# TongtongSong/OpenEAT

Measured on AMD Instinct MI355X. Metric: audio-frames/sec/GPU (train) + RTF (attention-rescoring decode), 12L Conformer, higher is better.
Workload: dtype f32 (storage, accumulate, softmax, norms, losses, optimizer all fp32; every matrix product is the fp32 product to within one fp32 rounding, computed as six exact bf16 x bf16 MFMA products of three-piece operand splits h+m+l = x, dropped terms < 2^-24 |a||b| - tests hold it to the exact-fp32 mode's t; 1 GPU; configs[1]: 12L Conformer d=256 (12+3+3, h=4, ff=1024, K=15, V=3246), B=32/GPU x 10 s 16 kHz wav (T=998 frames), L=30, CTC+attention joint loss, fbank+fwd+bwd+clip+Adam, dropout 0.1; global_batch=32, parallelism=dp1, hip_graph=True

## Files before the change

### include/openeat_hip.h

```cpp
#ifndef OPENEAT_HIP_H
#define OPENEAT_HIP_H

#include <stddef.h>
#include <stdint.h>

#ifdef __cplusplus
extern "C" {
#endif

const char* oe_last_error(void);
int oe_abi_version(void);

int oe_capture_unjoined_streams(void* origin, void* const* sides, int n_sides, int* unjoined_index);

int oe_stamp(long long* buf, int slot, void* stream);

enum { OE_GATHER_NONE = 0, OE_GATHER_A = 1, OE_GATHER_B = 2 };

typedef struct oe_gemm_args {
    const float* a; long lda; int a_kmajor;
    const float* b; long ldb; int b_kmajor;
    float* c; long ldc;
    int m, n, k;
    int split_k;
// ... 160 lines not shown
    const float* d_out;
    float* dq; float* dk; float* dv;
    float* dkeybias;
    float* delta;
    int precision;
    int causal;
} oe_attn_args;

int oe_attention_fwd(const oe_attn_args* args, void* stream);
int oe_attention_bwd(const oe_attn_args* args, void* stream);

int oe_relpos_prepare(const float* k, long k_bstride, long k_rstride, const float* p, long p_rstride,
                      const float* u, const float* v, int B, int T, int H, int D, float scale, float* kp,
                      float* keybias, void* stream);
int oe_relpos_backward(const float* dkp, const float* dkeybias, const float* k, long k_bstride, long k_rstride,
                       const float* p, long p_rstride, const float* u, const float* v, int B, int T, int H, int D,
                       float scale, float* dk, float* dp, long dp_rstride, float* du, float* dv, void* stream);

int oe_glu_fwd(const float* a, long rows, int d, float* y, void* stream);
int oe_glu_bwd(const float* a, const float* dy, long rows, int d, float* da, void* stream);

int oe_dropout_scale(const float* x, long n, int cols, float alpha, float p, unsigned long long seed,
                     const unsigned long long* seed_dev, const unsigned char* rowmask, float* out, void* stream);

int oe_embed_fwd(const long long* tokens, const float* table, const float* pe, long rows, int L, int d, int V,
                 float xscale, float* out, void* stream);
int oe_embed_bwd(const long long* tokens, const float* dout, long rows, int d, int V, float xscale, float* dtable,
                 void* stream);

int oe_swap_last2(const float* in, long A, int Bd, int Cd, float* out, int accumulate, void* stream);
int oe_pad1_nhwc(const float* dy, int B, int To, int Fo, int C, float* out, void* stream);
int oe_pad1_nhwc_planes(const float* dy, int B, int To, int Fo, int C, float* out, void* planes, long plane_stride, void* stream);
int oe_conv_dgrad_k3s2_weights(const float* w, int C, float* out, void* stream);

int oe_loss_combine(const float* loss_ctc, const float* loss_att, const float* loss_att_r, float ctc_weight, float reverse_weight,
                    float inv_accum, float* out, void* stream);
int oe_loss_combine_bwd(const float* g, float ctc_weight, float reverse_weight, float inv_accum, float* d_ctc, float* d_att,
                        float* d_att_r, void* stream);

int oe_axpby(const float* x, const float* y, long n, float a, float b, const float* a_dev, float* out, void* stream);

int oe_act_fwd(const float* x, long n, int act, float* y, void* stream);
int oe_act_grad(const float* dy, const float* pre, long n, int act, float* out, void* stream);

int oe_log_softmax(const float* x, long rows, int V, float* out, void* stream);
int oe_logprob_gather(const float* x, long rows, int V, const long long* idx_a, int idx_b, float* out_a, float* out_b, void* stream);
int oe_att_inputs(const int* ys_pad, const int* ys_lens, int B, int L, int sos, int eos, int ignore_id, long long* ys_in,
                  long long* ys_out, long long* r_ys_in, long long* r_ys_out, unsigned char* tgt_mask, void* stream);
int oe_topk_rows(const float* x, long rows, int V, int k, int log_softmax, float* vals, long long* idx, void* stream);

int oe_masked_softmax_fwd(const float* scores, const unsigned char* mask, long mask_bstride, long mask_rstride, int B, int H,
                          int T1, int T2, float drop_p, unsigned long long seed, const unsigned long long* seed_dev, float* y,
                          float* out, void* stream);
int oe_masked_softmax_bwd(const float* y, const float* dout, long rows, int T2, float drop_p, unsigned long long seed,
                          const unsigned long long* seed_dev, float* dscores, void* stream);

int oe_global_cmvn(const float* x, const float* mean, const float* istd, long n, int F, float* y, void* stream);

int oe_conv1_fwd(const float* x, const float* w, const float* bias, int B, int T, int F, int C, float* y, void* stream);
int oe_conv1_fwd_pl(const float* x, const float* w, const float* bias, int B, int T, int F, int C, float* y,
                    void* y_planes, long plane_stride, void* stream);
int oe_conv1_wgrad(const float* x, const float* dy, int B, int T, int F, int C, float* dw, float* db, void* stream);

int oe_col2im_relu(const float* dcol, const float* y1, int B, int T1, int F1, int C, float* dx, void* stream);
int oe_col2im_relu_ks(const float* dcol, const float* y1, int B, int T1, int F1, int C, int KS, int S, float* dx,
                      void* stream);
// ... 100 lines not shown
```

### openeat_amd/csrc/conv.hip

```cpp
#include <stdlib.h>
#include "oe_common.h"
#include "../../include/openeat_hip.h"

__global__ __launch_bounds__(256) void conv1_fwd_kernel(const float* __restrict__ x, const float* __restrict__ w,
                                                         const float* __restrict__ bias, int B, int T, int F, int T1, int F1,
                                                         int C, int pos_per_block, float* __restrict__ y,
                                                         __bf16* __restrict__ y_planes, long plane_stride) {
    const int cpt = C >> 2;
    const int grp = threadIdx.x / cpt;
    const int c4 = (threadIdx.x % cpt) * 4;
    const int ngrp = blockDim.x / cpt;
    float wr[4][9], br[4];
#pragma unroll
    for (int e = 0; e < 4; ++e) {
        br[e] = bias[c4 + e];
#pragma unroll
        for (int k = 0; k < 9; ++k) wr[e][k] = w[(c4 + e) * 9 + k];
    }
    const long npos = (long)B * T1 * F1;
    const long p0 = (long)blockIdx.x * pos_per_block;
    for (long pos = p0 + grp; pos < min(npos, p0 + pos_per_block); pos += ngrp) {
        const int f = (int)(pos % F1);
        const int t = (int)((pos / F1) % T1);
        const long b = pos / ((long)F1 * T1);
// ... 524 lines not shown
    hipLaunchKernelGGL(pad1_nhwc_planes_kernel, dim3((unsigned)min((long)oe_cdiv(n, 256), 65536L)), dim3(256), 0, (hipStream_t)stream,
                       (const float4*)dy, B, To, Fo, C / 4, (float4*)out, (__bf16*)planes, plane_stride);
    OE_LAUNCH_CHECK("pad1_nhwc_planes");
    return 0;
}
__global__ __launch_bounds__(256) void conv_dgrad_k3s2_weights_kernel(const float* __restrict__ w, int C, float* __restrict__ out) {
    const long n = 9L * C * C;
    const long i = (long)blockIdx.x * 256 + threadIdx.x;
    if (i >= n) return;
    const long cc = (long)C * C;
    int cls, KH, KW;
    long base;
    if (i < 4 * cc) { cls = 0; KH = 2; KW = 2; base = 0; }
    else if (i < 6 * cc) { cls = 1; KH = 2; KW = 1; base = 4 * cc; }
    else if (i < 8 * cc) { cls = 2; KH = 1; KW = 2; base = 6 * cc; }
    else { cls = 3; KH = 1; KW = 1; base = 8 * cc; }
    const long r = i - base;
    const int co = (int)(r % C);
    long q = r / C;
    const int kwi = (int)(q % KW);
    q /= KW;
    const int khi = (int)(q % KH);
    const int ci = (int)(q / KH);
    const int kh = (cls >> 1) ? 1 : (khi == 0 ? 2 : 0);
    const int kw = (cls & 1) ? 1 : (kwi == 0 ? 2 : 0);
    out[i] = w[(((long)co * C + ci) * 3 + kh) * 3 + kw];
}
extern "C" int oe_conv_dgrad_k3s2_weights(const float* w, int C, float* out, void* stream) {
    OE_REQUIRE(w && out && C > 0, "oe_conv_dgrad_k3s2_weights: bad arguments");
    hipLaunchKernelGGL(conv_dgrad_k3s2_weights_kernel, dim3(oe_cdiv(9L * C * C, 256)), dim3(256), 0, (hipStream_t)stream, w, C, out);
    OE_LAUNCH_CHECK("conv_dgrad_k3s2_weights");
    return 0;
}
```

### openeat_amd/csrc/gemm_pl.hip

```cpp
#include <stdlib.h>
#include "gemm_common.h"
#include "../../include/openeat_hip.h"

typedef __bf16 bf16x8 __attribute__((ext_vector_type(8)));
typedef __bf16 bf16x2 __attribute__((ext_vector_type(2)));
typedef short s16x4 __attribute__((ext_vector_type(4)));

struct PlOperand {
    const __bf16* p;
    long ld;
    long plane_stride;
    int rows_total;
    int T1, F1, T2, F2, C, KS, S;
    int korder, KH;
};

__device__ __forceinline__ void pl_dma16(const __bf16* src, unsigned dst) {
    unsigned keep;
    asm volatile("s_mov_b32 %0, m0\n\ts_mov_b32 m0, %2\n\ts_nop 0\n\tglobal_load_lds_dwordx4 %1, off\n\ts_mov_b32 m0, %0"
                 : "=&s"(keep) : "v"(src), "s"(dst) : "memory");
}
template <int N_OUTSTANDING>
__device__ __forceinline__ void pl_wait_and_barrier() {
    asm volatile("s_waitcnt vmcnt(%0)\n\ts_barrier" :: "n"(N_OUTSTANDING) : "memory");
// ... 21 lines not shown
    const unsigned char* p1 = tile + (kr0 + 4) * 256 + 16 * (ch ^ pl_gsw(kr0 + 4)) + 8 * (i & 1);
    typedef __attribute__((address_space(3))) s16x4 lds_s16x4;
#pragma unroll
    for (int n = 0; n < 3; ++n) {
        union { s16x4 h[2]; bf16x8 v; } u;
        u.h[0] = __builtin_amdgcn_ds_read_tr16_b64_v4i16((lds_s16x4*)(p0 + n * plane_bytes));
        u.h[1] = __builtin_amdgcn_ds_read_tr16_b64_v4i16((lds_s16x4*)(p1 + n * plane_bytes));
        f.p[n] = u.v;
    }
}

__device__ __forceinline__ float pl_frag_sum(const PlFrag& f, float c) {
    bf16x2 ones;
    ones[0] = (__bf16)1.0f; ones[1] = (__bf16)1.0f;
#pragma unroll
    for (int n = 0; n < 3; ++n) {
        union { bf16x8 v; bf16x2 q[4]; } u;
        u.v = f.p[n];
#pragma unroll
        for (int e = 0; e < 4; ++e) c = __builtin_amdgcn_fdot2_f32_bf16(u.q[e], ones, c, false);
    }
    return c;
}

__device__ __forceinline__ int pl_div_small(int k, int d, float rd, int& rem) {
    int q = (int)((float)k * rd);
    rem = k - q * d;
    if (rem >= d) { ++q; rem -= d; }
    if (rem < 0) { --q; rem += d; }
    return q;
}

template <int TM, int TN, int WM, bool AK, bool BKM, int BK, int NST, bool GA, bool GB>
__global__ __launch_bounds__(WM * 128, (WM == 2 && NST * 3 * (32 * TM * WM + 64 * TN) * BK * 2 <= 80 * 1024) ? 2 : (WM == 4 ? 2 : 1))
void gemm_pl_kernel(PlOperand A, PlOperand B, float* __restrict__ C, long ldc, int M, int N, int K, int k_chunk, int gx, int gy, EpiParams ep,
                    int k_valid, int m_base) {
    int tile_x, tile_y, tile_z;
    {
        const int nblk = gridDim.x, id = blockIdx.x;
        const int q = nblk >> 3, r = nblk & 7, xcd = id & 7, j = id >> 3;
        const int swz = (xcd < r ? xcd * (q + 1) : r * (q + 1) + (xcd - r) * q) + j;
        tile_x = swz % gx;
        tile_y = (swz / gx) % gy;
        tile_z = swz / (gx * gy);
    }
    constexpr int NW = WM * 2;
    constexpr int BM = 32 * TM * WM, BN = 64 * TN;
    static_assert(!AK || BM % 128 == 0, "k-major tiles are made of 128-column sub-tiles");
    static_assert(!BKM || BN % 128 == 0, "k-major tiles are made of 128-column sub-tiles");
    constexpr int A_T = BM * BK * 2, B_T = BN * BK * 2;
    constexpr int STAGE = 3 * (A_T + B_T);
    constexpr int PA = A_T / 1024, PB = B_T / 1024;
    constexpr int PTOT = 3 * (PA + PB), PPW = PTOT / NW;
    static_assert(PTOT % NW == 0 && A_T % 1024 == 0 && B_T % 1024 == 0, "piece count must split over the waves");
    constexpr int EPI_BYTES = NW * 32 * 36 * 4;
    constexpr int LDS_BYTES = (NST * STAGE > EPI_BYTES) ? NST * STAGE : EPI_BYTES;
    __shared__ __attribute__((aligned(1024))) unsigned char lds[LDS_BYTES];

    const int lane = threadIdx.x & 63;
    const int wave = __builtin_amdgcn_readfirstlane(threadIdx.x >> 6);
    const int wm = wave >> 1, wn = wave & 1;
    const long m0 = (long)m_base + (long)tile_y * BM, n0 = (long)tile_x * BN;
    const int k_begin = tile_z * k_chunk;
    const int k_end = min(K, k_begin + k_chunk);
    const int nk = (k_end - k_begin) / BK;

    const __bf16* src[PPW];
    unsigned dst[PPW];
    long step[PPW];
    int kpos[PPW];
    bool is_ga[PPW], is_gb[PPW];
    const float rF2 = GB ? 1.0f / (float)B.F2 : 0.f, rT2 = GB ? 1.0f / (float)B.T2 : 0.f;
#pragma unroll
    for (int j = 0; j < PPW; ++j) {
        const int g = wave * PPW + j;
        const bool isA = g < 3 * PA;
        const int gg = isA ? g : g - 3 * PA;
        const int P = isA ? PA : PB;
// ... 122 lines not shown
        };
        read_group(std::integral_constant<int, 0>{});
        begin_issue();
        static_for<0, NG>([&](auto gi) {
            constexpr int g = decltype(gi)::value;
            constexpr int ks = g / (TM * TN), i = (g / TN) % TM, j = g % TN;
            if constexpr (g + 1 < NG) read_group(std::integral_constant<int, g + 1>{});
            __builtin_amdgcn_sched_barrier(0);
            acc[i][j] = oe_mma_terms<6>(fa[ks][i], fb[ks][j], acc[i][j]);
            if (AK && j == 0 && do_csum) csum[i] = pl_frag_sum(fa[ks][i], csum[i]);
            __builtin_amdgcn_sched_barrier(0);
            static_for<0, PPG>([&](auto qi) {
                constexpr int pj = g * PPG + decltype(qi)::value;
                if constexpr (pj < PPW) issue_piece(pj);
            });
            __builtin_amdgcn_sched_barrier(0);
        });
        end_issue();
    }
    pl_wait_and_barrier<0>();
    if (AK && do_csum) {
        float al = ep.alpha;
        if (ep.alpha_dev) al *= *ep.alpha_dev;
#pragma unroll
        for (int i = 0; i < TM; ++i) {
            const float v = csum[i] + __shfl_xor(csum[i], 32, 64);
            const long row = m0 + wm * 32 * TM + i * 32 + frow;
            if (fhalf == 0 && row < M) atomicAdd(ep.a_colsum + row, v * al);
        }
    }
    gemm_epilogue<TM, TN, WM>(acc, reinterpret_cast<float*>(lds), C, ldc, M, N, m0, n0, ep, tile_z);
}

static long pl_launches = 0;
extern "C" long oe_gemm_pl_launches(void) { return pl_launches; }

static int pl_env(const char* name, int dflt) { const char* v = getenv(name); return v ? atoi(v) : dflt; }
static int pl_min_blocks = pl_env("OE_PL_MIN_BLOCKS", 96), pl_forced_tile = pl_env("OE_PL_TILE", 0), pl_forced_bk = pl_env("OE_PL_BK", 0),
           pl_waves = pl_env("OE_PL_WAVES", 8), pl_t44_min = pl_env("OE_PL_T44_MIN", 1024), pl_hybrid = pl_env("OE_PL_HYBRID", 1);
extern "C" int oe_gemm_pl_config(int min_blocks, int tile, int bk, int waves) {
    if (min_blocks >= 0) pl_min_blocks = min_blocks;
    if (tile >= 0) pl_forced_tile = tile;
    if (bk >= 0) pl_forced_bk = bk;
    if (waves >= 0) pl_waves = waves;
    return 0;
}

extern "C" int oe_gemm_pl_hybrid(int on) {
    const int was = pl_hybrid;
    if (on >= 0) pl_hybrid = on;
    return was;
}

static int pl_k_valid = 0;
template <int TM, int TN, int WM, bool AK, bool BKM, int BK, int NST, bool GA, bool GB>
static int launch_pl(const PlOperand& A_, const PlOperand& B, float* C, long ldc, int M, int N, int K, int sk, const EpiParams& ep, hipStream_t st,
                     int m_base = 0) {
    PlOperand A = A_;
    if (!AK) A.rows_total = M;
    int kc = oe_cdiv(oe_cdiv(K, sk), BK) * BK;
    if (kc <= 0) kc = BK;
    const int nz = oe_cdiv(K, kc);
    const int gx = oe_cdiv(N, 64 * TN), gy = oe_cdiv(M - m_base, 32 * TM * WM);
    hipLaunchKernelGGL((gemm_pl_kernel<TM, TN, WM, AK, BKM, BK, NST, GA, GB>), dim3(gx * gy * nz), dim3(WM * 128), 0, st, A, B, C, ldc, M, N, K, kc, gx, gy, ep,
                       pl_k_valid > 0 ? pl_k_valid : K, m_base);
    OE_LAUNCH_CHECK("oe_gemm (bf16x6 planes)");
// ... 72 lines not shown
        if (bk == 32) return launch_pl<2, 2, 2, AK, BKM, 32, 3, GA, GB>(a, b, C, ldc, M, N, K, sk, ep, st);           \
        return launch_pl<2, 2, 2, AK, BKM, 16, 3, GA, GB>(a, b, C, ldc, M, N, K, sk, ep, st);                         \
    } while (0)
    if (!a_kmajor && !b_kmajor) {
        if (tile == 11) return launch_pl<1, 1, 2, false, false, 32, 3, false, false>(a, b, C, ldc, M, N, K, sk, ep, st);
        if (tile == 24 && K % 32 == 0) {
            int m1 = 0;
            if (pl_hybrid && sk == 1 && !forced_tile && K % 16 == 0 && K >= 512 && M >= 256) {
                const int gxn = N / 256;
                const long t44 = (long)(M / 256) * gxn;
                const long full = t44 / 256;
                if (full >= 1 && (full * 256) % gxn == 0) {
                    const long rows1 = full * 256 / gxn * 256;
                    const long rest24 = (long)oe_cdiv(M - rows1, 128) * gxn;
                    const double cost_a = (double)oe_cdiv((long)oe_cdiv(M, 128) * gxn, 256L);
                    const double cost_b = 1.85 * full + (double)oe_cdiv(rest24, 256L);
                    if (rows1 < M && cost_b < cost_a) m1 = (int)rows1;
                }
            }
            if (m1 > 0) {
                if (ga) launch_pl<2, 4, 4, false, false, 16, 3, true, false>(a, b, C, ldc, m1, N, K, 1, ep, st);
                else launch_pl<2, 4, 4, false, false, 16, 3, false, false>(a, b, C, ldc, m1, N, K, 1, ep, st);
            }
            if (ga) return launch_pl<1, 4, 4, false, false, 32, 2, true, false>(a, b, C, ldc, M, N, K, sk, ep, st, m1);
            return launch_pl<1, 4, 4, false, false, 32, 2, false, false>(a, b, C, ldc, M, N, K, sk, ep, st, m1);
        }
        if (ga) OE_PL(false, false, true, false); else OE_PL(false, false, false, false);
    }
    if (!a_kmajor && b_kmajor) OE_PL(false, true, false, false);
    if (gb) OE_PL(true, true, false, true);
    OE_PL(true, true, false, false);
#undef OE_PL
}
```

### openeat_amd/hip.py

```python
from __future__ import annotations

import ctypes as C
import os
from typing import Optional

import torch

PROFILE = None

GEMM_PRECISION = int(os.environ.get("OE_GEMM_PRECISION", "0"))

_LIB_PATH = os.environ.get("OE_HIP_LIB") or os.path.join(os.path.dirname(os.path.abspath(__file__)), "lib", "libopeneat_hip.so")
_lib = None

ACT = {"none": 0, None: 0, "relu": 1, "swish": 2, "tanh": 3, "hardtanh": 4, "selu": 5, "gelu": 6}
GATHER_NONE, GATHER_A, GATHER_B = 0, 1, 2

c_fp = C.c_void_p


class GemmArgs(C.Structure):
    _fields_ = [
        ("a", c_fp), ("lda", C.c_long), ("a_kmajor", C.c_int),
        ("b", c_fp), ("ldb", C.c_long), ("b_kmajor", C.c_int),
# ... 96 lines not shown
        ("rowmask", c_fp),
        ("residual", c_fp), ("ldr", C.c_long), ("beta", C.c_float),
        ("y", c_fp), ("ldy", C.c_long),
        ("act", C.c_int), ("preact_out", c_fp), ("actgrad_in", c_fp), ("ld_aux", C.c_long),
        ("ln", LnPrologue), ("lnf", LnfPrologue), ("lne", LnEpilogue),
    ]


class HipLibraryMissing(RuntimeError):
    pass


def lib():
    global _lib
    if _lib is None:
        if not os.path.exists(_LIB_PATH):
            raise HipLibraryMissing(
                f"{_LIB_PATH} not found - build it with `python -c 'import __graft_entry__ as g; g.build()'` "
                "(openeat_amd has no CPU fallback)")
        _lib = C.CDLL(_LIB_PATH)
        _declare(_lib)
    return _lib


def exported_symbols():
    return list(_SIGNATURES)


class TnProblem(C.Structure):
    _fields_ = [("a", C.c_void_p), ("b", C.c_void_p), ("c", C.c_void_p), ("a_colsum", C.c_void_p), ("alpha_dev", C.c_void_p),
                ("lda", C.c_long), ("ldb", C.c_long), ("ldc", C.c_long), ("m", C.c_int), ("n", C.c_int), ("k", C.c_int),
                ("alpha", C.c_float), ("k_chunk", C.c_int), ("gx", C.c_int), ("gy", C.c_int), ("nz", C.c_int),
                ("block_start", C.c_int), ("reserved", C.c_int)]


class NgramModel(C.Structure):
    _fields_ = [("unigrams", c_fp), ("table", c_fp), ("tok2word", c_fp), ("capacity", C.c_long), ("n_words", C.c_int),
                ("max_probe", C.c_int), ("order", C.c_int), ("bos_word", C.c_int), ("eos_word", C.c_int), ("unk_word", C.c_int),
                ("V", C.c_int)]


class ContextGraph(C.Structure):
    _fields_ = [("edges", c_fp), ("fail", c_fp), ("out", c_fp), ("pend", c_fp), ("capacity", C.c_long), ("max_probe", C.c_int),
                ("n_states", C.c_int), ("c", C.c_float)]


class PrefixBeamArgs(C.Structure):
    _fields_ = [("topk_logp", c_fp), ("topk_idx", c_fp), ("lens", c_fp),
                ("B", C.c_int), ("Tmax", C.c_int), ("beam", C.c_int), ("max_len", C.c_int),
                ("lm", C.POINTER(NgramModel)), ("ctx", C.POINTER(ContextGraph)),
                ("lm_weight", C.c_double), ("length_bonus", C.c_double), ("eos", C.c_int), ("final", C.c_int),
                ("workspace", c_fp), ("out_prefix", c_fp), ("out_len", c_fp),
                ("out_score", c_fp), ("out_ctc", c_fp), ("out_lm", c_fp), ("out_bias", c_fp)]


I, L, F, D, P, U64, SZ = C.c_int, C.c_long, C.c_float, C.c_double, c_fp, C.c_ulonglong, C.c_size_t
_SIGNATURES = {
    "oe_last_error": (C.c_char_p, []),
    "oe_abi_version": (I, []),
    "oe_capture_unjoined_streams": (I, [P, C.POINTER(C.c_void_p), I, C.POINTER(I)]),
    "oe_stamp": (I, [P, I, P]),
    "oe_gemm_f32": (I, [C.POINTER(GemmArgs), P]),
    "oe_split_planes": (I, [P, L, L, L, P, L, L, P]),
    "oe_gemm_pl_launches": (L, []),
    "oe_gemm_hyb_launches": (L, []),
    "oe_gemm_pl_config": (I, [I, I, I, I]),
# ... 14 lines not shown
    "oe_rowgemm6_form": (I, [I, I, I]),
    "oe_colsum_f32": (I, [P, L, I, I, F, P, P, I, P]),
    "oe_layernorm_fwd": (I, [P, P, P, F, I, I, P, I, P, P, P]),
    "oe_layernorm_fwd_pl": (I, [P, P, P, F, I, I, P, I, P, P, P, L, P]),
    "oe_layernorm_bwd_workspace_floats": (SZ, [I, I]),
    "oe_layernorm_pair_fwd": (I, [P, P, P, F, P, P, F, I, I, P, P, P, P, P]),
    "oe_layernorm_pair_bwd_dx_drop": (I, [P, P, P, P, P, P, P, I, I, P, P, P, F, F, U64, P, P, P, P, P]),
    "oe_layernorm_bwd": (I, [P, P, P, P, I, P, I, I, P, P, P, P, P, P, P]),
    "oe_layernorm_bwd_dx": (I, [P, P, P, P, I, P, I, I, P, P, P, P, P]),
    "oe_layernorm_param_reduce": (I, [P, I, I, P, P, P]),
    "oe_layernorm_param_reduce_table": (I, [P, I, I, I, P]),
    "oe_layernorm_bwd_dx_drop": (I, [P, P, P, P, I, P, I, I, P, P, P, P, F, F, U64, P, P, P, P]),
    "oe_layernorm_bwd_dx_drop_pl": (I, [P, P, P, P, I, P, I, I, P, P, P, P, F, F, U64, P, P, P, P, L, P]),
    "oe_ctc_workspace_floats": (SZ, [I, I, I]),
    "oe_ctc_config": (I, [I, I]),
    "oe_ctc_loss_fused": (I, [P, L, I, I, I, P, P, I, P, F, P, P, P, P, P, P]),
    "oe_ctc_loss_fused_stats": (I, [P, L, I, I, I, P, P, I, P, F, P, P, P, P, P, P, I, P]),
    "oe_ctc_greedy": (I, [P, L, I, I, I, P, I, P, P, P, P]),
    "oe_ctc_align_workspace_bytes": (SZ, [I, I, I]),
    "oe_ctc_align": (I, [P, L, I, I, I, P, P, I, P, P, P, P, P, P, P, P]),
    "oe_attention_fwd": (I, [C.POINTER(AttnArgs), P]),
    "oe_attention_bwd": (I, [C.POINTER(AttnArgs), P]),
    "oe_relpos_prepare": (I, [P, L, L, P, L, P, P, I, I, I, I, F, P, P, P]),
    "oe_relpos_backward": (I, [P, P, P, L, L, P, L, P, P, I, I, I, I, F, P, P, L, P, P, P]),
    "oe_glu_fwd": (I, [P, L, I, P, P]),
    "oe_glu_bwd": (I, [P, P, L, I, P, P]),
    "oe_dropout_scale": (I, [P, L, I, F, F, U64, P, P, P, P]),
    "oe_embed_fwd": (I, [P, P, P, L, I, I, I, F, P, P]),
    "oe_embed_bwd": (I, [P, P, L, I, I, F, P, P]),
    "oe_swap_last2": (I, [P, L, I, I, P, I, P]),
    "oe_pad1_nhwc": (I, [P, I, I, I, I, P, P]),
    "oe_pad1_nhwc_planes": (I, [P, I, I, I, I, P, P, L, P]),
    "oe_conv_dgrad_k3s2_weights": (I, [P, I, P, P]),
    "oe_axpby": (I, [P, P, L, F, F, P, P, P]),
    "oe_loss_combine": (I, [P, P, P, F, F, F, P, P]),
    "oe_loss_combine_bwd": (I, [P, F, F, F, P, P, P, P]),
    "oe_act_fwd": (I, [P, L, I, P, P]),
    "oe_act_grad": (I, [P, P, L, I, P, P]),
    "oe_log_softmax": (I, [P, L, I, P, P]),
    "oe_topk_rows": (I, [P, L, I, I, I, P, P, P]),
    "oe_logprob_gather": (I, [P, L, I, P, I, P, P, P]),
    "oe_att_inputs": (I, [P, P, I, I, I, I, I, P, P, P, P, P, P]),
    "oe_masked_softmax_fwd": (I, [P, P, L, L, I, I, I, I, F, U64, P, P, P, P]),
    "oe_masked_softmax_bwd": (I, [P, P, L, I, F, U64, P, P, P]),
    "oe_global_cmvn": (I, [P, P, P, L, I, P, P]),
    "oe_conv1_fwd": (I, [P, P, P, I, I, I, I, P, P]),
    "oe_conv1_fwd_pl": (I, [P, P, P, I, I, I, I, P, P, L, P]),
    "oe_conv1_wgrad": (I, [P, P, I, I, I, I, P, P, P]),
    "oe_col2im_relu": (I, [P, P, I, I, I, I, P, P]),
    "oe_col2im_relu_ks": (I, [P, P, I, I, I, I, I, I, P, P]),
    "oe_dwconv_glu_fwd": (I, [P, P, P, P, I, I, I, I, I, P, P]),
    "oe_dwconv_glu_ln_fwd": (I, [P, P, P, P, I, I, I, I, I, P, P, P, F, I, P, P, P]),
    "oe_dwconv_glu_bwd_workspace_floats": (SZ, [I, I, I, I]),
    "oe_dwconv_glu_bwd": (I, [P, P, P, P, I, I, I, I, I, P, P, P, P, P, P]),
    "oe_lsm_workspace_bytes": (SZ, [L]),
    "oe_lsm_loss_fused": (I, [P, L, L, I, P, I, F, I, F, F, I, P, P, P]),
    "oe_fbank": (I, [P, P, I, L, I, I, I, I, F, F, P, P, P, P, P, F, P, P, P, P]),
    "oe_fbank_dither": (I, [P, P, I, L, I, I, I, I, F, F, P, P, P, P, P, F, P, P, F, U64, P, P]),
    "oe_utt_normalize": (I, [P, P, I, I, I, P]),
    "oe_spec_augment": (I, [P, P, I, I, I, P, I, P, I, F, P]),
    "oe_spec_substitute": (I, [P, I, I, I, P, I, I, P]),
    "oe_feature_dither": (I, [P, P, I, I, I, F, U64, P]),
    "oe_speed_perturb": (I, [P, L, P, P, I, I, P, L, P, P]),
    "oe_ctc_prefix_beam_workspace_bytes": (SZ, [I, I, I]),
    "oe_ctc_prefix_beam": (I, [C.POINTER(PrefixBeamArgs), P]),
    "oe_ctc_prefix_beam_host": (I, [P, P, I, I, I, P, P, P]),
# ... 68 lines not shown
    g.residual = None if residual is None else residual.data_ptr()
    g.ldr, g.beta, g.res_row_mod = ldr, beta, res_row_mod
    g.accumulate, g.atomic_out = int(accumulate), int(atomic_out)
    g.conv_gather = conv_gather
    g.precision = GEMM_PRECISION if precision is None else precision
    g.a_colsum = None if (a_colsum is None or g.precision == 0) else a_colsum.data_ptr()
    g.conv_kh = conv_kh
    g.conv_korder = conv_korder
    if g.precision == 6:
        if a_planes is not None and b_planes is not None:
            g.a_planes, g.a_plane_stride = a_planes.ptr, a_planes.stride
            g.b_planes, g.b_plane_stride = b_planes.ptr, b_planes.stride
            g.planes_k_padded = int(a_kmajor and b_kmajor and getattr(a_planes, "kpad", False) and getattr(b_planes, "kpad", False))
        elif b_planes is not None and a is not None:
            g.b_planes, g.b_plane_stride = b_planes.ptr, b_planes.stride
        if c_planes is not None:
            g.c_planes, g.c_plane_stride, g.ldcp = c_planes.ptr, c_planes.stride, c_planes.ld
    if scatter is not None:
        g.out_scatter = 1
        g.sc_t1, g.sc_f1, g.sc_t2, g.sc_f2, g.sc_s = scatter
    if conv is not None:
        g.conv_t1, g.conv_f1, g.conv_t2, g.conv_f2, g.conv_c = conv[:5]
        g.conv_k, g.conv_s = (conv[5], conv[6]) if len(conv) > 5 else (0, 0)
    if PROFILE is not None:
        e0, e1 = torch.cuda.Event(enable_timing=True), torch.cuda.Event(enable_timing=True)
        e0.record()
        check(lib().oe_gemm_f32(C.byref(g), stream()), "oe_gemm_f32")
        e1.record()
        PROFILE.append((e0, e1, 2.0 * m * n * k, (m, n, k, int(a_kmajor), int(b_kmajor), int(conv_gather), int(split_k))))
        return
    check(lib().oe_gemm_f32(C.byref(g), stream()), "oe_gemm_f32")


def tn_grouped_plan(problems, target_blocks: int = 384):
    n = len(problems)
    arr = (TnProblem * n)()
    dp = lambda t: None if t is None else t.data_ptr()
    for i, q in enumerate(problems):
        dy, x, out = q["dy"], q["x"], q["out"]
        p = arr[i]
        p.a, p.b, p.c, p.a_colsum, p.alpha_dev = dy.data_ptr(), x.data_ptr(), out.data_ptr(), dp(q.get("bias_out")), dp(q.get("alpha_dev"))
        p.lda, p.ldb, p.ldc = dy.stride(0), x.stride(0), out.stride(0)
        p.m, p.n, p.k, p.alpha = dy.shape[1], x.shape[1], dy.shape[0], float(q.get("alpha", 1.0))
    total = lib().oe_gemm_tn_grouped_plan(arr, n, int(target_blocks))
    if total < 0:
        return None
    return bytes(arr), total


def tn_grouped_launch(table_dev: torch.Tensor, n: int, total_blocks: int, precision=None, flops: float = 0.0):
    if PROFILE is not None:
        e0, e1 = torch.cuda.Event(enable_timing=True), torch.cuda.Event(enable_timing=True)
        e0.record()
        check(lib().oe_gemm_tn_grouped(C.c_void_p(table_dev.data_ptr()), n, total_blocks, GEMM_PRECISION if precision is None else precision,
                                       stream()), "oe_gemm_tn_grouped")
        e1.record()
        PROFILE.append((e0, e1, flops, ("tn_grouped", n, total_blocks, 0, 1, 1, 0)))
        return
    check(lib().oe_gemm_tn_grouped(C.c_void_p(table_dev.data_ptr()), n, total_blocks, GEMM_PRECISION if precision is None else precision,
                                   stream()), "oe_gemm_tn_grouped")


def ffn_fwd(x2, w1p, b1, w2p, b2, rows, d, ff, act, *, drop_in=0.0, seed_in=0, drop_out=0.0, seed_out=0, seed_dev=None, pre_out=None,
            act_out=None, residual=None, ldr=0, beta=1.0, y=None, precision=None, lnf=None):
    a = FfnArgs()
    dp = lambda t: None if t is None else t.data_ptr()
# ... 227 lines not shown
```

### openeat_amd/ops.py

```python
from __future__ import annotations

import itertools
import os
import math
import weakref
from typing import Optional

import torch

from . import hip
from . import arena as _arena
from . import planes as _planes

ACT_NONE, ACT_RELU, ACT_SWISH, ACT_TANH, ACT_HARDTANH, ACT_SELU, ACT_GELU = 0, 1, 2, 3, 4, 5, 6
ACT_IDS = {"relu": ACT_RELU, "swish": ACT_SWISH, "tanh": ACT_TANH, "hardtanh": ACT_HARDTANH, "selu": ACT_SELU, "gelu": ACT_GELU,
           "none": ACT_NONE}
GEMM_FUSED_ACTS = (ACT_NONE, ACT_RELU, ACT_SWISH)


_seed_counter = itertools.count(0x5EED0001)
_seed_dev: Optional[torch.Tensor] = None


def next_seed() -> int:
# ... 1637 lines not shown
        dgpad = torch.zeros(d, device=dy.device) if causal else None
        ws = _new(hip.lib().oe_dwconv_glu_bwd_workspace_floats(B, T, d, K), like=dy)
        hip.call("oe_dwconv_glu_bwd", a, dyc, wd, gpad, B, T, d, K, int(causal), da, dwd, dbd, dgpad, ws)
        (db1, rb1) = grad_sink(b1)
        tw1 = _arena.grad_target(w1)
        ow1 = tw1.view(2 * d, d) if tw1 is not None else _new(2 * d, d, like=dy, zero=True)
        pl = wgrad_planes(da, xm)
        _run_wgrad(tw1 is not None and rb1 is None and not causal, (da, xm) + _pl_tensors(pl), lambda: gemm_tn(da, xm, out=ow1, bias_out=db1, planes=pl),
                   desc=dict(dy=da, x=xm, out=ow1, alpha=1.0, alpha_dev=None, bias_out=db1))
        dw1 = None if tw1 is not None else ow1.view(w1.shape)
        if causal:
            db1_pad = torch.empty_like(db1)
            hip.call("oe_glu_bwd", b1, dgpad, 1, d, db1_pad)
            hip.call("oe_axpby", db1_pad, db1, 2 * d, 1.0, 1.0, None, db1)
        dx = gemm_nn(da, w1m, rowmask=rowmask).view(B, T, d)
        return dx, None, dw1, rb1, rwd, rbd, rg, rbeta, dw2, db2, None, None, None, (dy if has_res else None), None, None


def conv_module(x, rowmask, w1, b1, wd, bd, g, b, w2, b2, K, causal, act, residual=None, p_out=0.0, input_masked=False):
    return ConvModuleFn.apply(x, rowmask, w1, b1, wd, bd, g, b, w2, b2, K, causal, act, residual, p_out, input_masked)


CONV_DGRAD_IMPLICIT = os.environ.get("OE_CONV_DGRAD", "implicit") != "col2im"
CONV_KORDER = os.environ.get("OE_CONV_KORDER", "1") == "1"
CONV_KORDER_MIN_ROWS = 32768


def _korder_cols(w2d, taps, C):
    r = w2d.shape[0]
    return w2d.view(r, taps, C // 32, 32).permute(0, 2, 1, 3).contiguous().view(r, taps * C)
CONV_WGRAD_PLANES = os.environ.get("OE_CONV_WGRAD_PLANES", "1") == "1"
CONV1_PLANES_ONLY = os.environ.get("OE_CONV1_PLANES_ONLY", "1") == "1"
CONV_PAD_PLANES = os.environ.get("OE_CONV_PAD_PLANES", "1") == "1"


def _conv_dgrad_k3s2(dy, wk, yin, B, Ti, Fi, To, Fo, C, yin_planes=None):
    ni_min, nj_min = Ti // 2, Fi // 2
    direct = bool(_planes.available() and CONV_PAD_PLANES and CONV_KORDER and C % 32 == 0 and B * ni_min * nj_min >= CONV_KORDER_MIN_ROWS)
    dyp_pl = None
    if direct:
        dyp = None
        dyp_pl = _planes.alloc(B * (To + 2) * (Fo + 2), C, dy.device)
        hip.call("oe_pad1_nhwc_planes", dy, B, To, Fo, C, None, dyp_pl.t, dyp_pl.stride)
    else:
        dyp = _new(B, To + 2, Fo + 2, C, like=dy)
        hip.call("oe_pad1_nhwc", dy, B, To, Fo, C, dyp)
    wcls = _new(9 * C * C, like=dy)
    hip.call("oe_conv_dgrad_k3s2_weights", wk, C, wcls)
    dyin = torch.empty_like(yin) if yin_planes is None else _new(B, Ti, Fi, C, like=dy)
    flat_in, flat_out = (None if dyp is None else dyp.view(-1)), dyin.view(-1)
    flat_y = yin.reshape(-1) if yin_planes is None else yin_planes.t[0].reshape(-1)
    if dyp_pl is None:
        dyp_pl = _planes.of(dyp.view(-1, C)) if _planes.available() else None
    w_off = 0
    for pt in (0, 1):
        KH = 2 if pt == 0 else 1
        ni = (Ti + 1 - pt) // 2
        for pf in (0, 1):
            KW = 2 if pf == 0 else 1
            nj = (Fi + 1 - pf) // 2
            wsel = wcls[w_off:w_off + KH * KW * C * C].view(C, KH * KW * C)
            w_off += KH * KW * C * C
            a_off = (pt * (Fo + 2) + pf) * C
            o_off = (pt * Fi + pf) * C
            ap = bp = None
            korder = 0
            if dyp_pl is not None:
                korder = int(CONV_KORDER and C % 32 == 0 and B * ni * nj >= CONV_KORDER_MIN_ROWS)
                bp = _planes.of(_korder_cols(wsel, KH * KW, C) if korder else wsel, force=True)
                if bp is not None:
                    ap = _planes.Planes(dyp_pl.t, dyp_pl.ptr + 2 * a_off, dyp_pl.stride, C, dyp_pl.rows, C)
                else:
                    korder = 0
            assert flat_in is not None or (korder and ap is not None)
            hip.gemm(None if flat_in is None else flat_in[a_off:], wsel, flat_out[o_off:], B * ni * nj, C, KH * KW * C, lda=0, ldb=KH * KW * C, ldc=C,
                     act=ACT_RELU, actgrad_in=flat_y[o_off:], ld_aux=C, conv=(To + 2, Fo + 2, ni, nj, C, KW, 1), conv_gather=hip.GATHER_A,
                     conv_kh=KH, scatter=(Ti, Fi, ni, nj, 2), a_planes=ap, b_planes=bp, conv_korder=korder, actgrad_bf16=yin_planes is not None)
    return dyin


class ConvSubsamplingFn(torch.autograd.Function):

    @staticmethod
    def forward(ctx, x, w1, b1, wl, bl, pe, xscale, geoms, *stage_params):
# ... 431 lines not shown
```

Before: 2.003 million audio-frames/s.

## Group the four stride-2 conv dgrad parity classes into one planes GEMM launch

Adds a grouped implicit-GEMM kernel that runs all four parity classes of the k3s2 conv data-gradient in one launch (or two, for the hybrid big/small tile split). Each block finds its class from a tile-start table with XCD-aware local indexing. A new kernel writes the reordered weights straight into bf16 split planes, replacing the fp32 weight shuffle and the per-class plane conversions. The aim is to cut launch count, per-class planes passes and tail underutilization in conv subsampling backward, at the cost of a more complex scheduler and a separate code path.

```diff
diff --git a/include/openeat_hip.h b/include/openeat_hip.h
--- a/include/openeat_hip.h
+++ b/include/openeat_hip.h
@@ -216,6 +216,22 @@
 int oe_pad1_nhwc(const float* dy, int B, int To, int Fo, int C, float* out, void* stream);
 int oe_pad1_nhwc_planes(const float* dy, int B, int To, int Fo, int C, float* out, void* planes, long plane_stride, void* stream);
 int oe_conv_dgrad_k3s2_weights(const float* w, int C, float* out, void* stream);
+int oe_conv_dgrad_k3s2_weight_planes(const float* w, int C, void* planes, long plane_stride, void* stream);
+
+typedef struct oe_dgrad_class {
+    const void* b_planes;
+    long a_off, o_off, m_off;
+    int kh, kw, ni, nj;
+} oe_dgrad_class;
+typedef struct oe_dgrad_grouped_args {
+    const void* dy_planes; long dy_plane_stride;
+    long b_plane_stride;
+    float* out; const void* mask; int mask_bf16;
+    int B, Ti, Fi, To, Fo, C;
+    int n_classes;
+    oe_dgrad_class cls[4];
+} oe_dgrad_grouped_args;
+int oe_conv_dgrad_k3s2_grouped(const oe_dgrad_grouped_args* args, void* stream);
 
 int oe_loss_combine(const float* loss_ctc, const float* loss_att, const float* loss_att_r, float ctc_weight, float reverse_weight,
                     float inv_accum, float* out, void* stream);
diff --git a/openeat_amd/csrc/conv.hip b/openeat_amd/csrc/conv.hip
--- a/openeat_amd/csrc/conv.hip
+++ b/openeat_amd/csrc/conv.hip
@@ -580,3 +580,37 @@
     OE_LAUNCH_CHECK("conv_dgrad_k3s2_weights");
     return 0;
 }
+__global__ __launch_bounds__(256) void conv_dgrad_k3s2_weight_planes_kernel(const float* __restrict__ w, int C, __bf16* __restrict__ planes, long pstride) {
+    const long cc = (long)C * C;
+    const long i = ((long)blockIdx.x * 256 + threadIdx.x) * 4;
+    if (i >= 9 * cc) return;
+    int cls, KH, KW;
+    long base;
+    if (i < 4 * cc) { cls = 0; KH = 2; KW = 2; base = 0; }
+    else if (i < 6 * cc) { cls = 1; KH = 2; KW = 1; base = 4 * cc; }
+    else if (i < 8 * cc) { cls = 2; KH = 1; KW = 2; base = 6 * cc; }
+    else { cls = 3; KH = 1; KW = 1; base = 8 * cc; }
+    const int taps = KH * KW;
+    const long r = i - base;
+    const int c32 = (int)(r % 32);
+    long q = r / 32;
+    const int tap = (int)(q % taps);
+    q /= taps;
+    const int chunk = (int)(q % (C / 32));
+    const int ci = (int)(q / (C / 32));
+    const int khi = tap / KW, kwi = tap - khi * KW;
+    const int kh = (cls >> 1) ? 1 : (khi == 0 ? 2 : 0);
+    const int kw = (cls & 1) ? 1 : (kwi == 0 ? 2 : 0);
+    const float* src = w + (((long)(chunk * 32 + c32) * C + ci) * 3 + kh) * 3 + kw;
+    const long co_stride = (long)C * 9;
+    store_planes4(planes + i, pstride, make_float4(src[0], src[co_stride], src[2 * co_stride], src[3 * co_stride]));
+}
+extern "C" int oe_conv_dgrad_k3s2_weight_planes(const float* w, int C, void* planes, long plane_stride, void* stream) {
+    OE_REQUIRE(w && planes && C > 0 && C % 32 == 0, "oe_conv_dgrad_k3s2_weight_planes: bad arguments (C must be a multiple of 32)");
+    OE_REQUIRE((((uintptr_t)planes) & 7) == 0 && plane_stride % 4 == 0 && plane_stride >= 9L * C * C,
+               "oe_conv_dgrad_k3s2_weight_planes: planes must be 8-byte aligned, the plane stride a multiple of 4 and at least 9 C^2");
+    hipLaunchKernelGGL(conv_dgrad_k3s2_weight_planes_kernel, dim3(oe_cdiv(9L * C * C / 4, 256)), dim3(256), 0, (hipStream_t)stream, w, C,
+                       (__bf16*)planes, plane_stride);
+    OE_LAUNCH_CHECK("conv_dgrad_k3s2_weight_planes");
+    return 0;
+}
diff --git a/openeat_amd/csrc/gemm_pl.hip b/openeat_amd/csrc/gemm_pl.hip
--- a/openeat_amd/csrc/gemm_pl.hip
+++ b/openeat_amd/csrc/gemm_pl.hip
@@ -77,18 +77,8 @@
 }
 
 template <int TM, int TN, int WM, bool AK, bool BKM, int BK, int NST, bool GA, bool GB>
-__global__ __launch_bounds__(WM * 128, (WM == 2 && NST * 3 * (32 * TM * WM + 64 * TN) * BK * 2 <= 80 * 1024) ? 2 : (WM == 4 ? 2 : 1))
-void gemm_pl_kernel(PlOperand A, PlOperand B, float* __restrict__ C, long ldc, int M, int N, int K, int k_chunk, int gx, int gy, EpiParams ep,
-                    int k_valid, int m_base) {
-    int tile_x, tile_y, tile_z;
-    {
-        const int nblk = gridDim.x, id = blockIdx.x;
-        const int q = nblk >> 3, r = nblk & 7, xcd = id & 7, j = id >> 3;
-        const int swz = (xcd < r ? xcd * (q + 1) : r * (q + 1) + (xcd - r) * q) + j;
-        tile_x = swz % gx;
-        tile_y = (swz / gx) % gy;
-        tile_z = swz / (gx * gy);
-    }
+__device__ __forceinline__ void pl_tile(const PlOperand& A, const PlOperand& B, float* __restrict__ C, long ldc, int M, int N, int K, int k_chunk,
+                                        int tile_x, int tile_y, int tile_z, const EpiParams& ep, int k_valid, int m_base) {
     constexpr int NW = WM * 2;
     constexpr int BM = 32 * TM * WM, BN = 64 * TN;
     static_assert(!AK || BM % 128 == 0, "k-major tiles are made of 128-column sub-tiles");
@@ -277,6 +267,63 @@
     gemm_epilogue<TM, TN, WM>(acc, reinterpret_cast<float*>(lds), C, ldc, M, N, m0, n0, ep, tile_z);
 }
 
+#define PL_LAUNCH_BOUNDS(TM, TN, WM, BK, NST) \
+    __launch_bounds__(WM * 128, (WM == 2 && NST * 3 * (32 * TM * WM + 64 * TN) * BK * 2 <= 80 * 1024) ? 2 : (WM == 4 ? 2 : 1))
+
+template <int TM, int TN, int WM, bool AK, bool BKM, int BK, int NST, bool GA, bool GB>
+__global__ PL_LAUNCH_BOUNDS(TM, TN, WM, BK, NST)
+void gemm_pl_kernel(PlOperand A, PlOperand B, float* __restrict__ C, long ldc, int M, int N, int K, int k_chunk, int gx, int gy, EpiParams ep,
+                    int k_valid, int m_base) {
+    const int nblk = gridDim.x, id = blockIdx.x;
+    const int q = nblk >> 3, r = nblk & 7, xcd = id & 7, j = id >> 3;
+    const int swz = (xcd < r ? xcd * (q + 1) : r * (q + 1) + (xcd - r) * q) + j;
+    pl_tile<TM, TN, WM, AK, BKM, BK, NST, GA, GB>(A, B, C, ldc, M, N, K, k_chunk, swz % gx, (swz / gx) % gy, swz / (gx * gy), ep, k_valid, m_base);
+}
+
+struct PlGroupClass {
+    const __bf16* a;
+    const __bf16* b;
+    float* c;
+    const void* aux;
+    int K, KH, KW;
+    int T2, F2;
+    int m_base, m_end;
+    int tile_start;
+};
+struct PlGroup {
+    PlGroupClass cls[4];
+    int n, n_tiles;
+    long a_pstride, b_pstride;
+    int T1, F1, C;
+    int sc_t1, sc_f1;
+    int aux_bf16;
+};
+
+template <int TM, int TN, int WM, int BK, int NST>
+__global__ PL_LAUNCH_BOUNDS(TM, TN, WM, BK, NST)
+void gemm_pl_grouped_kernel(PlGroup g) {
+    const int id = blockIdx.x;
+    int p = 0;
+#pragma unroll
+    for (int q = 1; q < 4; ++q) if (q < g.n && g.cls[q].tile_start <= id) p = q;
+    const PlGroupClass c = g.cls[p];
+    const int s = c.tile_start, e = (p + 1 < g.n) ? g.cls[(p + 1) & 3].tile_start : g.n_tiles;
+    const int x = id & 7;
+    auto below = [x](int t) { return (t >> 3) * x + min(t & 7, x); };
+    const int local = below(e) - below(s) + ((id - (s + ((x - s) & 7))) >> 3);
+    constexpr int BN = 64 * TN;
+    const int gx = (g.C + BN - 1) / BN;
+    PlOperand A{}, B{};
+    A.p = c.a; A.plane_stride = g.a_pstride; A.rows_total = c.m_end;
+    A.T1 = g.T1; A.F1 = g.F1; A.T2 = c.T2; A.F2 = c.F2; A.C = g.C; A.KS = c.KW; A.S = 1; A.korder = 1; A.KH = c.KH;
+    B.p = c.b; B.ld = c.K; B.plane_stride = g.b_pstride; B.rows_total = g.C;
+    EpiParams ep{};
+    ep.alpha = 1.f; ep.beta = 1.f; ep.act = OE_ACT_RELU; ep.actgrad_in = reinterpret_cast<const float*>(c.aux); ep.ld_aux = g.C;
+    ep.actgrad_bf16 = g.aux_bf16; ep.ldr = g.C; ep.ld_cp = g.C;
+    ep.scatter = 1; ep.sc_t1 = g.sc_t1; ep.sc_f1 = g.sc_f1; ep.sc_t2 = c.T2; ep.sc_f2 = c.F2; ep.sc_s = 2;
+    pl_tile<TM, TN, WM, false, false, BK, NST, true, false>(A, B, c.c, g.C, c.m_end, g.C, c.K, c.K, local % gx, local / gx, 0, ep, c.K, c.m_base);
+}
+
 static long pl_launches = 0;
 extern "C" long oe_gemm_pl_launches(void) { return pl_launches; }
 
@@ -415,3 +462,102 @@
     OE_PL(true, true, false, false);
 #undef OE_PL
 }
+
+static int pl_grp_big_min_k = pl_env("OE_PL_GROUPED_BIG_MIN_K", 512);
+
+template <int TM, int TN, int WM, int BK, int NST>
+static int launch_pl_grouped(PlGroup& g, const long (&m_base)[4], const long (&m_end)[4], hipStream_t st) {
+    PlGroup q = g;
+    constexpr int BM = 32 * TM * WM, BN = 64 * TN;
+    const int gx = oe_cdiv(g.C, BN);
+    long tiles = 0;
+    q.n = 0;
+    for (int i = 0; i < g.n; ++i) {
+        if (m_end[i] <= m_base[i]) continue;
+        PlGroupClass& c = q.cls[q.n++];
+        c = g.cls[i];
+        c.m_base = (int)m_base[i]; c.m_end = (int)m_end[i]; c.tile_start = (int)tiles;
+        tiles += (long)oe_cdiv(m_end[i] - m_base[i], BM) * gx;
+    }
+    if (q.n == 0) return 0;
+    OE_REQUIRE(tiles < (1L << 30), "oe_conv_dgrad_k3s2_grouped: too many tiles");
+    q.n_tiles = (int)tiles;
+    hipLaunchKernelGGL((gemm_pl_grouped_kernel<TM, TN, WM, BK, NST>), dim3((unsigned)tiles), dim3(WM * 128), 0, st, q);
+    OE_LAUNCH_CHECK("oe_conv_dgrad_k3s2_grouped");
+    ++pl_launches;
+    return 0;
+}
+
+extern "C" int oe_conv_dgrad_k3s2_grouped(const oe_dgrad_grouped_args* a, void* stream) {
+    OE_REQUIRE(a && a->dy_planes && a->out && a->mask, "oe_conv_dgrad_k3s2_grouped: null argument");
+    const int C = a->C;
+    OE_REQUIRE(a->B > 0 && a->Ti >= 3 && a->Fi >= 3 && a->To == (a->Ti - 3) / 2 + 1 && a->Fo == (a->Fi - 3) / 2 + 1 && C > 0 && C % 32 == 0,
+               "oe_conv_dgrad_k3s2_grouped: bad geometry (B=%d Ti=%d Fi=%d To=%d Fo=%d C=%d; C must be a multiple of 32)", a->B, a->Ti, a->Fi, a->To, a->Fo, C);
+    OE_REQUIRE(a->n_classes >= 1 && a->n_classes <= 4, "oe_conv_dgrad_k3s2_grouped: 1 to 4 classes");
+    OE_REQUIRE((((uintptr_t)a->dy_planes | (uintptr_t)a->out) & 15) == 0 && a->dy_plane_stride % 8 == 0 && a->b_plane_stride % 8 == 0 &&
+                   (((uintptr_t)a->mask) & (a->mask_bf16 ? 7 : 15)) == 0,
+               "oe_conv_dgrad_k3s2_grouped: dy planes / out / mask must be 16-byte (a bf16 mask: 8-byte) aligned, plane strides multiples of 8");
+    const long T1 = a->To + 2, F1 = a->Fo + 2;
+    OE_REQUIRE(a->dy_plane_stride >= (long)a->B * T1 * F1 * C, "oe_conv_dgrad_k3s2_grouped: dy plane stride shorter than the padded dy");
+    PlGroup g{};
+    g.a_pstride = a->dy_plane_stride; g.b_pstride = a->b_plane_stride;
+    g.T1 = (int)T1; g.F1 = (int)F1; g.C = C; g.sc_t1 = a->Ti; g.sc_f1 = a->Fi; g.aux_bf16 = a->mask_bf16 != 0;
+    int order[4], n = a->n_classes;
+    for (int i = 0; i < n; ++i) {
+        int j = i;
+        for (; j > 0 && a->cls[order[j - 1]].kh * a->cls[order[j - 1]].kw < a->cls[i].kh * a->cls[i].kw; --j) order[j] = order[j - 1];
+        order[j] = i;
+    }
+    long rows[4];
+    for (int i = 0; i < n; ++i) {
+        const oe_dgrad_class& s = a->cls[order[i]];
+        OE_REQUIRE(s.b_planes && (((uintptr_t)s.b_planes) & 15) == 0 && (s.kh == 1 || s.kh == 2) && (s.kw == 1 || s.kw == 2) && s.ni >= 1 && s.nj >= 1,
+                   "oe_conv_dgrad_k3s2_grouped: class %d: bad window / null or unaligned B planes", order[i]);
+        OE_REQUIRE(a->b_plane_stride >= (long)C * s.kh * s.kw * C, "oe_conv_dgrad_k3s2_grouped: class %d: B plane stride shorter than the operand", order[i]);
+        OE_REQUIRE(s.a_off >= 0 && s.a_off % C == 0 && s.o_off >= 0 && s.o_off % C == 0 && s.m_off >= 0 && s.m_off % C == 0,
+                   "oe_conv_dgrad_k3s2_grouped: class %d: offsets must be whole positions", order[i]);
+        const long ar = s.a_off / C / F1, ac = s.a_off / C % F1, orow = s.o_off / C / a->Fi, oc = s.o_off / C % a->Fi;
+        OE_REQUIRE(ar + s.ni - 1 + s.kh - 1 < T1 && ac + s.nj - 1 + s.kw - 1 < F1, "oe_conv_dgrad_k3s2_grouped: class %d: window leaves the padded dy", order[i]);
+        OE_REQUIRE(orow + 2L * (s.ni - 1) < a->Ti && oc + 2L * (s.nj - 1) < a->Fi && s.m_off == s.o_off,
+                   "oe_conv_dgrad_k3s2_grouped: class %d: scattered rows leave the output (or the mask offset differs from the output's)", order[i]);
+        rows[i] = (long)a->B * s.ni * s.nj;
+        OE_REQUIRE(rows[i] < (1L << 31) - 256, "oe_conv_dgrad_k3s2_grouped: class %d: too many rows", order[i]);
+        PlGroupClass& c = g.cls[i];
+        c.a = (const __bf16*)a->dy_planes + s.a_off;
+        c.b = (const __bf16*)s.b_planes;
+        c.c = a->out + s.o_off;
+        c.aux = a->mask_bf16 ? (const void*)((const __bf16*)a->mask + s.m_off) : (const void*)((const float*)a->mask + s.m_off);
+        c.KH = s.kh; c.KW = s.kw; c.K = s.kh * s.kw * C; c.T2 = s.ni; c.F2 = s.nj;
+    }
+    g.n = n;
+    hipStream_t st = (hipStream_t)stream;
+    const long zero[4] = {0, 0, 0, 0};
+    const int forced = pl_forced_tile;
+    OE_REQUIRE(forced == 0 || forced == 22 || forced == 24 || forced == 44, "oe_conv_dgrad_k3s2_grouped: forced tile %d is not one of 22 / 24 / 44", forced);
+    if (C % 256 != 0 || forced == 22) return launch_pl_grouped<1, 2, 4, 32, 3>(g, zero, rows, st);
+    if (forced == 44) return launch_pl_grouped<2, 4, 4, 16, 3>(g, zero, rows, st);
+    long m1[4] = {0, 0, 0, 0};
+    if (pl_hybrid && !forced) {
+        const int gxn = C / 256;
+        long t44 = 0, all24 = 0;
+        for (int i = 0; i < n; ++i) {
+            if (g.cls[i].K >= pl_grp_big_min_k) t44 += rows[i] / 256 * gxn;
+            all24 += (long)oe_cdiv(rows[i], 128) * gxn;
+        }
+        const long full = t44 / 256;
+        if (full >= 1 && (full * 256) % gxn == 0) {
+            long left = full * 256 / gxn, rest24 = 0;
+            for (int i = 0; i < n; ++i) {
+                const long take = g.cls[i].K >= pl_grp_big_min_k ? min(rows[i] / 256, left) : 0;
+                left -= take;
+                m1[i] = take * 256;
+                rest24 += (long)oe_cdiv(rows[i] - m1[i], 128) * gxn;
+            }
+            if (!(1.85 * full + (double)oe_cdiv(rest24, 256L) < (double)oe_cdiv(all24, 256L)))
+                for (int i = 0; i < n; ++i) m1[i] = 0;
+        }
+    }
+    const int r = launch_pl_grouped<2, 4, 4, 16, 3>(g, zero, m1, st);
+    if (r) return r;
+    return launch_pl_grouped<1, 4, 4, 32, 2>(g, m1, rows, st);
+}
diff --git a/openeat_amd/hip.py b/openeat_amd/hip.py
--- a/openeat_amd/hip.py
+++ b/openeat_amd/hip.py
@@ -152,6 +152,18 @@
                 ("lda", C.c_long), ("ldb", C.c_long), ("ldc", C.c_long), ("m", C.c_int), ("n", C.c_int), ("k", C.c_int),
                 ("alpha", C.c_float), ("k_chunk", C.c_int), ("gx", C.c_int), ("gy", C.c_int), ("nz", C.c_int),
                 ("block_start", C.c_int), ("reserved", C.c_int)]
+
+
+class DgradClass(C.Structure):
+    _fields_ = [("b_planes", c_fp), ("a_off", C.c_long), ("o_off", C.c_long), ("m_off", C.c_long),
+                ("kh", C.c_int), ("kw", C.c_int), ("ni", C.c_int), ("nj", C.c_int)]
+
+
+class DgradGroupedArgs(C.Structure):
+    _fields_ = [("dy_planes", c_fp), ("dy_plane_stride", C.c_long), ("b_plane_stride", C.c_long),
+                ("out", c_fp), ("mask", c_fp), ("mask_bf16", C.c_int),
+                ("B", C.c_int), ("Ti", C.c_int), ("Fi", C.c_int), ("To", C.c_int), ("Fo", C.c_int), ("C", C.c_int),
+                ("n_classes", C.c_int), ("cls", DgradClass * 4)]
 
 
 class NgramModel(C.Structure):
@@ -232,6 +244,8 @@
     "oe_pad1_nhwc": (I, [P, I, I, I, I, P, P]),
     "oe_pad1_nhwc_planes": (I, [P, I, I, I, I, P, P, L, P]),
     "oe_conv_dgrad_k3s2_weights": (I, [P, I, P, P]),
+    "oe_conv_dgrad_k3s2_weight_planes": (I, [P, I, P, L, P]),
+    "oe_conv_dgrad_k3s2_grouped": (I, [C.POINTER(DgradGroupedArgs), P]),
     "oe_axpby": (I, [P, P, L, F, F, P, P, P]),
     "oe_loss_combine": (I, [P, P, P, F, F, F, P, P]),
     "oe_loss_combine_bwd": (I, [P, F, F, F, P, P, P, P]),
@@ -366,6 +380,26 @@
     check(lib().oe_gemm_f32(C.byref(g), stream()), "oe_gemm_f32")
 
 
+def conv_dgrad_grouped(dy_planes, classes, out, mask, mask_bf16, B, Ti, Fi, To, Fo, Cc, b_plane_stride):
+    a = DgradGroupedArgs()
+    a.dy_planes, a.dy_plane_stride, a.b_plane_stride = dy_planes.ptr, dy_planes.stride, b_plane_stride
+    a.out, a.mask, a.mask_bf16 = out.data_ptr(), mask.data_ptr(), int(mask_bf16)
+    a.B, a.Ti, a.Fi, a.To, a.Fo, a.C = B, Ti, Fi, To, Fo, Cc
+    a.n_classes = len(classes)
+    flops = 0.0
+    for s, (bp, a_off, o_off, kh, kw, ni, nj) in zip(a.cls, classes):
+        s.b_planes, s.a_off, s.o_off, s.m_off, s.kh, s.kw, s.ni, s.nj = bp, a_off, o_off, o_off, kh, kw, ni, nj
+        flops += 2.0 * B * ni * nj * Cc * kh * kw * Cc
+    if PROFILE is not None:
+        e0, e1 = torch.cuda.Event(enable_timing=True), torch.cuda.Event(enable_timing=True)
+        e0.record()
+        check(lib().oe_conv_dgrad_k3s2_grouped(C.byref(a), stream()), "oe_conv_dgrad_k3s2_grouped")
+        e1.record()
+        PROFILE.append((e0, e1, flops, ("conv_dgrad_grouped", B * Ti * Fi, Cc, 9 * Cc // 4, 0, 0, 1, 1)))
+        return
+    check(lib().oe_conv_dgrad_k3s2_grouped(C.byref(a), stream()), "oe_conv_dgrad_k3s2_grouped")
+
+
 def tn_grouped_plan(problems, target_blocks: int = 384):
     n = len(problems)
     arr = (TnProblem * n)()
diff --git a/openeat_amd/ops.py b/openeat_amd/ops.py
--- a/openeat_amd/ops.py
+++ b/openeat_amd/ops.py
@@ -1693,6 +1693,7 @@
 CONV_WGRAD_PLANES = os.environ.get("OE_CONV_WGRAD_PLANES", "1") == "1"
 CONV1_PLANES_ONLY = os.environ.get("OE_CONV1_PLANES_ONLY", "1") == "1"
 CONV_PAD_PLANES = os.environ.get("OE_CONV_PAD_PLANES", "1") == "1"
+CONV_DGRAD_GROUPED = os.environ.get("OE_CONV_DGRAD_GROUPED", "1") == "1"
 
 
 def _conv_dgrad_k3s2(dy, wk, yin, B, Ti, Fi, To, Fo, C, yin_planes=None):
@@ -1706,11 +1707,25 @@
     else:
         dyp = _new(B, To + 2, Fo + 2, C, like=dy)
         hip.call("oe_pad1_nhwc", dy, B, To, Fo, C, dyp)
-    wcls = _new(9 * C * C, like=dy)
-    hip.call("oe_conv_dgrad_k3s2_weights", wk, C, wcls)
+    grouped = direct and CONV_DGRAD_GROUPED
+    if grouped:
+        wpl = torch.empty(3, 9 * C * C, dtype=torch.bfloat16, device=dy.device)
+        hip.call("oe_conv_dgrad_k3s2_weight_planes", wk, C, wpl, 9 * C * C)
+    else:
+        wcls = _new(9 * C * C, like=dy)
+        hip.call("oe_conv_dgrad_k3s2_weights", wk, C, wcls)
     dyin = torch.empty_like(yin) if yin_planes is None else _new(B, Ti, Fi, C, like=dy)
     flat_in, flat_out = (None if dyp is None else dyp.view(-1)), dyin.view(-1)
     flat_y = yin.reshape(-1) if yin_planes is None else yin_planes.t[0].reshape(-1)
+    if grouped:
+        classes, w_off = [], 0
+        for pt in (0, 1):
+            for pf in (0, 1):
+                KH, KW = 2 - pt, 2 - pf
+                classes.append((wpl.data_ptr() + 2 * w_off, (pt * (Fo + 2) + pf) * C, (pt * Fi + pf) * C, KH, KW, (Ti + 1 - pt) // 2, (Fi + 1 - pf) // 2))
+                w_off += KH * KW * C * C
+        hip.conv_dgrad_grouped(dyp_pl, classes, flat_out, flat_y, yin_planes is not None, B, Ti, Fi, To, Fo, C, 9 * C * C)
+        return dyin
     if dyp_pl is None:
         dyp_pl = _planes.of(dyp.view(-1, C)) if _planes.available() else None
     w_off = 0
```

Result: no change. 2.022 million audio-frames/s (median of 6 runs) (+0.9%).
